# evgueni-ovtchinnikov/raleigh

Hardware: AMD Instinct MI355X
Metric: inner-iter GB/s vs HBM roofline (Gram+dots+SpMM of one block-JCG iteration) (higher is better)
Workload: dtype f64; 1 GPU; block-JCG inner iteration: 9 Gram + 4 dots + 1 SpMM, n=215x215x215=9938375 rows (9938375 per GPU), m=32, 7-pt Laplacian nnz=69291275, rows sharded over 1 GPU(s), strong scaling; n=9938375, m=32, nnz=69291275

## Files before the change

include/rlhip.h:

```cpp
#ifndef RLHIP_H
#define RLHIP_H

#include <stdint.h>

#ifdef __cplusplus
extern "C" {
#endif

#define RLH_VERSION 100

enum { RLH_S = 0, RLH_D = 1, RLH_C = 2, RLH_Z = 3 };

int rlh_version(void);
const char *rlh_last_error(void);
int rlh_device_count(int *count);
int rlh_init(int device);
int rlh_finalize(void);
int rlh_set_stream(void *hip_stream);
int rlh_sync(void);
int rlh_mem_info(int64_t *free_bytes, int64_t *total_bytes);

int rlh_malloc(void **dptr, int64_t bytes);
int rlh_free(void *dptr);
int rlh_memset(void *dptr, int value, int64_t bytes);
int rlh_h2d(void *dptr, const void *hptr, int64_t bytes);
int rlh_d2h(void *hptr, const void *dptr, int64_t bytes);
int rlh_d2d(void *dst, const void *src, int64_t bytes);
int rlh_fetch(void *hptr, const void *dptr, int64_t bytes);
int rlh_copy2d(void *dst, int64_t dpitch, const void *src, int64_t spitch,
               int64_t width_bytes, int64_t rows, int kind);

int rlh_gram(int dtype, int64_t n, int64_t mx, const void *X, int64_t ldx,
             int64_t my, const void *Y, int64_t ldy, void *d_out, void *h_out);

int rlh_gram_multi(int dtype, int64_t n, int nx, const void *const *X, const int64_t *ldx,
                   const int64_t *mx, int ny, const void *const *Y, const int64_t *ldy,
                   const int64_t *my, void *d_out, void *h_out);

int rlh_dots(int dtype, int64_t n, int64_t m, const void *X, int64_t ldx,
             const void *Y, int64_t ldy, void *d_out, void *h_out);

int rlh_dots_transp(int dtype, int64_t n, int64_t m, const void *X, int64_t ldx,
                    const void *Y, int64_t ldy, void *d_out);
int rlh_absmax(int dtype, int64_t n, int64_t m, const void *X, int64_t ldx, double *h_out);

int rlh_block_update(int dtype, int64_t n, int64_t k, const void *X, int64_t ldx,
                     int64_t m, void *Out, int64_t ldo, const void *q,
                     int64_t q_rs, int64_t q_cs, const double *alpha, int beta);

int rlh_block_update2(int dtype, int64_t n, int64_t k1, const void *X1, int64_t ldx1,
                      const void *q1, int64_t q1_rs, int64_t q1_cs, int64_t k2,
                      const void *X2, int64_t ldx2, const void *q2, int64_t q2_rs,
                      int64_t q2_cs, int64_t m, void *Out, int64_t ldo,
                      const double *alpha, int beta);
int rlh_block_update2x2(int dtype, int64_t n, int64_t k1, const void *X1, int64_t ldx1,
                        const void *q1, int64_t q1_rs, int64_t q1_cs, int64_t k2, const void *X2,
                        int64_t ldx2, const void *q2, int64_t q2_rs, int64_t q2_cs, int64_t ma,
                        void *OutA, int64_t ldoa, int64_t mb, void *OutB, int64_t ldob);
int rlh_lincomb_cols(int dtype, int64_t n, int64_t m, const void *a, const void *A,
                     int64_t lda, const void *b, const void *B, int64_t ldb, void *Out,
                     int64_t ldo);
// ... 112 lines not shown
```

raleigh_amd/_lib.py:

```python

import ctypes
import os

import numpy as np

_PKG = os.path.dirname(os.path.abspath(__file__))
LIBPATH = os.path.join(_PKG, 'lib', 'librlhip.so')

RLH_S, RLH_D, RLH_C, RLH_Z = 0, 1, 2, 3

DTYPE_CODE = {np.float32: RLH_S, np.float64: RLH_D, np.complex64: RLH_C, np.complex128: RLH_Z}
DTYPE_SIZE = {np.float32: 4, np.float64: 8, np.complex64: 8, np.complex128: 16}

_i64 = ctypes.c_int64
_p = ctypes.c_void_p
_int = ctypes.c_int

SIGNATURES = {
    'rlh_version': [],
    'rlh_last_error': [],
    'rlh_device_count': [ctypes.POINTER(_int)],
    'rlh_init': [_int],
    'rlh_finalize': [],
    'rlh_set_stream': [_p],
    'rlh_sync': [],
    'rlh_mem_info': [ctypes.POINTER(_i64), ctypes.POINTER(_i64)],
    'rlh_malloc': [ctypes.POINTER(_p), _i64],
    'rlh_free': [_p],
    'rlh_memset': [_p, _int, _i64],
    'rlh_h2d': [_p, _p, _i64],
    'rlh_d2h': [_p, _p, _i64],
    'rlh_d2d': [_p, _p, _i64],
    'rlh_fetch': [_p, _p, _i64],
    'rlh_copy2d': [_p, _i64, _p, _i64, _i64, _i64, _int],
    'rlh_gram': [_int, _i64, _i64, _p, _i64, _i64, _p, _i64, _p, _p],
    'rlh_gram_multi': [_int, _i64, _int, _p, _p, _p, _int, _p, _p, _p, _p, _p],
    'rlh_dots': [_int, _i64, _i64, _p, _i64, _p, _i64, _p, _p],
    'rlh_absmax': [_int, _i64, _i64, _p, _i64, ctypes.POINTER(ctypes.c_double)],
    'rlh_dots_transp': [_int, _i64, _i64, _p, _i64, _p, _i64, _p],
    'rlh_block_update': [_int, _i64, _i64, _p, _i64, _i64, _p, _i64, _p, _i64, _i64, _p, _int],
    'rlh_block_update2': [_int, _i64, _i64, _p, _i64, _p, _i64, _i64, _i64, _p, _i64, _p, _i64, _i64, _i64, _p, _i64,
                          _p, _int],
    'rlh_block_update2x2': [_int, _i64, _i64, _p, _i64, _p, _i64, _i64, _i64, _p, _i64, _p, _i64, _i64, _i64, _p, _i64,
                            _i64, _p, _i64],
    'rlh_lincomb_cols': [_int, _i64, _i64, _p, _p, _i64, _p, _p, _i64, _p, _i64],
    'rlh_axpy': [_int, _i64, _i64, _p, _p, _i64, _p, _i64],
    'rlh_axpy_cols': [_int, _i64, _i64, _p, _p, _i64, _p, _i64],
    'rlh_copy': [_int, _i64, _i64, _p, _i64, _p, _i64],
    'rlh_copy_cols': [_int, _i64, _i64, _p, _p, _i64, _p, _i64],
    'rlh_scale_cols': [_int, _i64, _i64, _p, _int, _p, _i64],
    'rlh_convert': [_int, _int, _i64, _i64, _p, _i64, _p, _i64],
    'rlh_fill_random': [_int, _i64, _i64, _p, _i64, ctypes.c_uint64, _i64, _i64],
    'rlh_conj': [_int, _i64, _i64, _p, _i64],
    'rlh_gather_rows': [_int, _i64, _p, _i64, _p, _i64, _p, _i64],
    'rlh_csr_create': [ctypes.POINTER(_p), _int, _i64, _i64, _p, _p, _p],
    'rlh_csr_create_upper': [ctypes.POINTER(_p), _int, _i64, _p, _p, _p],
    'rlh_csr_destroy': [_p],
    'rlh_csr_info': [_p, ctypes.POINTER(_i64), ctypes.POINTER(_i64), ctypes.POINTER(_i64),
                     ctypes.POINTER(_i64)],
    'rlh_csr_layout': [_p, ctypes.POINTER(_int), ctypes.POINTER(_i64), ctypes.POINTER(ctypes.c_double)],
    'rlh_csr_stacks': [_p, ctypes.POINTER(_i64), ctypes.POINTER(ctypes.c_double), ctypes.POINTER(ctypes.c_double)],
    'rlh_csr_bf16_ready': [_p, _i64, _i64, ctypes.POINTER(_int)],
    'rlh_spmm': [_p, _i64, _p, _i64, _i64, _p, _i64, _p, _i64],
    'rlh_spmm_cheb': [_p, _i64, _p, _i64, _i64, _p, _i64, _p, _i64, _p, _i64, ctypes.c_double, ctypes.c_double,
                      ctypes.c_double],
    'rlh_spmm_part': [_p, _int, _i64, _p, _i64, _i64, _p, _i64, _p, _i64],
# ... 118 lines not shown
```

raleigh_amd/csrc/common.h:

```cpp
#pragma once

#include <hip/hip_runtime.h>
#include <stdint.h>
#include <stdio.h>
#include <string.h>

#include <stdlib.h>

#include <string>
#include <thread>
#include <vector>

#include "rlhip.h"

namespace rlh {

void set_error(const char *fmt, ...);
int hip_fail(hipError_t e, const char *what, const char *file, int line);

#define RLH_HIP(call)                                                   \
  do {                                                                  \
    hipError_t e_ = (call);                                             \
    if (e_ != hipSuccess) return rlh::hip_fail(e_, #call, __FILE__, __LINE__); \
  } while (0)
// ... 64 lines not shown
__device__ __forceinline__ float  add_of(float a, float b)   { return a + b; }
__device__ __forceinline__ double add_of(double a, double b) { return a + b; }
__device__ __forceinline__ c32 add_of(c32 a, c32 b) { return c32{a.re + b.re, a.im + b.im}; }
__device__ __forceinline__ c64 add_of(c64 a, c64 b) { return c64{a.re + b.re, a.im + b.im}; }
__device__ __forceinline__ float  mul_of(float a, float b)   { return a * b; }
__device__ __forceinline__ double mul_of(double a, double b) { return a * b; }
__device__ __forceinline__ c32 mul_of(c32 a, c32 b) { return c32{a.re * b.re - a.im * b.im, a.re * b.im + a.im * b.re}; }
__device__ __forceinline__ c64 mul_of(c64 a, c64 b) { return c64{a.re * b.re - a.im * b.im, a.re * b.im + a.im * b.re}; }

constexpr int kRingSlots = 16;
constexpr size_t kRingSlotBytes = 1u << 20;
constexpr size_t kWorkspaceBytes = 96u << 20;

struct Context {
  bool ready = false;
  int device = -1;
  int num_cu = 256;
  hipStream_t own_stream = nullptr;
  hipStream_t stream = nullptr;
  char *ring_h = nullptr;
  char *ring_d = nullptr;
  hipEvent_t ring_ev[kRingSlots];
  bool ring_used[kRingSlots];
  int ring_next = 0;
  char *work = nullptr;
  char *result_d = nullptr;
  size_t result_d_bytes = 0;
  char *result_h = nullptr;
  char *result_hd = nullptr;
  size_t result_h_bytes = 0;
  hipEvent_t t0 = nullptr, t1 = nullptr;
  unsigned *async_err_h = nullptr;
  unsigned *async_err_d = nullptr;
};

Context &ctx();
int require_ready();
int check_async_error();

int ring_acquire(size_t bytes, int *slot, void **h, void **d);
int ring_commit(int slot, size_t bytes);
int ring_release(int slot);

int ensure_result(size_t bytes);
int fetch_result(void *h_out, const void *d_src, size_t bytes);

static inline bool aligned16(const void *p, int64_t ld, int64_t es) {
  return ((reinterpret_cast<uintptr_t>(p) & 15u) == 0) && (((ld * es) & 15) == 0);
}

}
```

raleigh_amd/csrc/context.hip:

```cpp
#include <stdarg.h>

#include "common.h"

namespace rlh {

static thread_local char g_err[1024] = "";

void set_error(const char *fmt, ...) {
  va_list ap;
  va_start(ap, fmt);
  vsnprintf(g_err, sizeof(g_err), fmt, ap);
  va_end(ap);
}

int hip_fail(hipError_t e, const char *what, const char *file, int line) {
  set_error("hip error %d (%s) in %s at %s:%d", (int)e, hipGetErrorString(e), what, file, line);
  return (int)e ? (int)e : 1;
}

int host_threads() {
  int t = env_int("RLH_HOST_THREADS", 0);
  if (t <= 0) {
    t = (int)std::thread::hardware_concurrency();
    if (t > 16) t = 16;
  }
  return t < 1 ? 1 : t;
}

Context &ctx() {
  static Context c;
  return c;
}

// ... 14 lines not shown
  }
  return 0;
}

int ring_acquire(size_t bytes, int *slot, void **h, void **d) {
  Context &c = ctx();
  RLH_REQUIRE(bytes <= kRingSlotBytes, "coefficient block of %zu bytes exceeds the %zu-byte staging slot",
              bytes, kRingSlotBytes);
  int s = c.ring_next;
  c.ring_next = (s + 1) % kRingSlots;
  if (c.ring_used[s]) RLH_HIP(hipEventSynchronize(c.ring_ev[s]));
  *slot = s;
  *h = c.ring_h + (size_t)s * kRingSlotBytes;
  *d = c.ring_d + (size_t)s * kRingSlotBytes;
  return 0;
}

int ring_commit(int slot, size_t bytes) {
  Context &c = ctx();
  RLH_HIP(hipMemcpyAsync(c.ring_d + (size_t)slot * kRingSlotBytes, c.ring_h + (size_t)slot * kRingSlotBytes,
                         bytes, hipMemcpyHostToDevice, c.stream));
  return 0;
}

int ring_release(int slot) {
  Context &c = ctx();
  RLH_HIP(hipEventRecord(c.ring_ev[slot], c.stream));
  c.ring_used[slot] = true;
  return 0;
}

int ensure_result(size_t bytes) {
  Context &c = ctx();
  if (bytes > c.result_d_bytes) {
    size_t nb = bytes < (1u << 20) ? (1u << 20) : bytes * 2;
    RLH_HIP(hipStreamSynchronize(c.stream));
    if (c.result_d) RLH_HIP(hipFree(c.result_d));
    if (c.result_h) RLH_HIP(hipHostFree(c.result_h));
    c.result_d = nullptr; c.result_h = nullptr; c.result_hd = nullptr; c.result_d_bytes = c.result_h_bytes = 0;
    RLH_HIP(hipMalloc((void **)&c.result_d, nb));
    RLH_HIP(hipHostMalloc((void **)&c.result_h, nb, hipHostMallocMapped));
    RLH_HIP(hipHostGetDevicePointer((void **)&c.result_hd, c.result_h, 0));
    c.result_d_bytes = c.result_h_bytes = nb;
  }
  return 0;
}

int fetch_result(void *h_out, const void *d_src, size_t bytes) {
  Context &c = ctx();
  if (bytes == 0) return 0;
  if (d_src == c.result_hd && bytes <= c.result_h_bytes) {
    RLH_HIP(hipStreamSynchronize(c.stream));
    memcpy(h_out, c.result_h, bytes);
  } else if (bytes <= c.result_h_bytes) {
    RLH_HIP(hipMemcpyAsync(c.result_h, d_src, bytes, hipMemcpyDeviceToHost, c.stream));
    RLH_HIP(hipStreamSynchronize(c.stream));
    memcpy(h_out, c.result_h, bytes);
  } else {
    RLH_HIP(hipMemcpyAsync(h_out, d_src, bytes, hipMemcpyDeviceToHost, c.stream));
    RLH_HIP(hipStreamSynchronize(c.stream));
  }
  return check_async_error();
}

}

using namespace rlh;

extern "C" {

int rlh_version(void) { return RLH_VERSION; }

const char *rlh_last_error(void) { return g_err; }

int rlh_device_count(int *count) {
  RLH_REQUIRE(count != nullptr, "rlh_device_count: null argument");
  RLH_HIP(hipGetDeviceCount(count));
  return 0;
}

int rlh_init(int device) {
  Context &c = ctx();
  if (c.ready) {
    RLH_REQUIRE(c.device == device, "rlh_init: already bound to device %d (one device per process)", c.device);
    return 0;
  }
  int count = 0;
  RLH_HIP(hipGetDeviceCount(&count));
  RLH_REQUIRE(device >= 0 && device < count, "rlh_init: device %d out of range (%d visible)", device, count);
  RLH_HIP(hipSetDevice(device));
  hipDeviceProp_t prop;
  RLH_HIP(hipGetDeviceProperties(&prop, device));
  RLH_REQUIRE(strncmp(prop.gcnArchName, "gfx950", 6) == 0,
              "rlh_init: device %d is %s; this library is built for gfx950 (MI355X) only", device, prop.gcnArchName);
  c.num_cu = prop.multiProcessorCount;
  RLH_HIP(hipStreamCreateWithFlags(&c.own_stream, hipStreamNonBlocking));
  c.stream = c.own_stream;
  RLH_HIP(hipHostMalloc((void **)&c.ring_h, kRingSlots * kRingSlotBytes, hipHostMallocDefault));
  RLH_HIP(hipMalloc((void **)&c.ring_d, kRingSlots * kRingSlotBytes));
  for (int i = 0; i < kRingSlots; ++i) {
    RLH_HIP(hipEventCreateWithFlags(&c.ring_ev[i], hipEventDisableTiming));
    c.ring_used[i] = false;
  }
  RLH_HIP(hipMalloc((void **)&c.work, kWorkspaceBytes));
  RLH_HIP(hipEventCreate(&c.t0));
  RLH_HIP(hipEventCreate(&c.t1));
  RLH_HIP(hipHostMalloc((void **)&c.async_err_h, 64, hipHostMallocMapped));
  *c.async_err_h = 0;
  RLH_HIP(hipHostGetDevicePointer((void **)&c.async_err_d, c.async_err_h, 0));
  c.device = device;
  c.ready = true;
  if (int rc = ensure_result(1u << 20)) return rc;
  return 0;
}

int rlh_finalize(void) {
  Context &c = ctx();
  if (!c.ready) return 0;
  (void)hipStreamSynchronize(c.stream);
  for (int i = 0; i < kRingSlots; ++i) (void)hipEventDestroy(c.ring_ev[i]);
  (void)hipEventDestroy(c.t0);
  (void)hipEventDestroy(c.t1);
  (void)hipHostFree(c.ring_h);
  (void)hipFree(c.ring_d);
  (void)hipFree(c.work);
  if (c.result_d) (void)hipFree(c.result_d);
  if (c.result_h) (void)hipHostFree(c.result_h);
  if (c.async_err_h) (void)hipHostFree(c.async_err_h);
  (void)hipStreamDestroy(c.own_stream);
  c = Context();
  return 0;
}

int rlh_set_stream(void *hip_stream) {
  if (int rc = require_ready()) return rc;
  Context &c = ctx();
  RLH_HIP(hipStreamSynchronize(c.stream));
  c.stream = hip_stream ? (hipStream_t)hip_stream : c.own_stream;
  return 0;
}

int rlh_sync(void) {
  if (int rc = require_ready()) return rc;
  RLH_HIP(hipStreamSynchronize(ctx().stream));
  return check_async_error();
}

int rlh_mem_info(int64_t *free_bytes, int64_t *total_bytes) {
  if (int rc = require_ready()) return rc;
  size_t f = 0, t = 0;
  RLH_HIP(hipMemGetInfo(&f, &t));
  if (free_bytes) *free_bytes = (int64_t)f;
  if (total_bytes) *total_bytes = (int64_t)t;
  return 0;
}

int rlh_malloc(void **dptr, int64_t bytes) {
  if (int rc = require_ready()) return rc;
  RLH_REQUIRE(dptr != nullptr && bytes >= 0, "rlh_malloc: bad arguments");
  *dptr = nullptr;
  if (bytes == 0) return 0;
// ... 8 lines not shown
  RLH_HIP(hipFree(dptr));
  return 0;
}

int rlh_memset(void *dptr, int value, int64_t bytes) {
  if (int rc = require_ready()) return rc;
  if (bytes <= 0) return 0;
  RLH_HIP(hipMemsetAsync(dptr, value, (size_t)bytes, ctx().stream));
  return 0;
}

int rlh_h2d(void *dptr, const void *hptr, int64_t bytes) {
  if (int rc = require_ready()) return rc;
  if (bytes <= 0) return 0;
  RLH_HIP(hipMemcpyAsync(dptr, hptr, (size_t)bytes, hipMemcpyHostToDevice, ctx().stream));
  RLH_HIP(hipStreamSynchronize(ctx().stream));
  return 0;
}

int rlh_d2h(void *hptr, const void *dptr, int64_t bytes) {
  if (int rc = require_ready()) return rc;
  if (bytes <= 0) return 0;
  RLH_HIP(hipMemcpyAsync(hptr, dptr, (size_t)bytes, hipMemcpyDeviceToHost, ctx().stream));
  RLH_HIP(hipStreamSynchronize(ctx().stream));
  return 0;
}

int rlh_fetch(void *hptr, const void *dptr, int64_t bytes) {
  if (int rc = require_ready()) return rc;
  if (bytes <= 0) return 0;
  RLH_REQUIRE(hptr && dptr, "rlh_fetch: null pointer");
  if (int rc = ensure_result((size_t)bytes)) return rc;
  return fetch_result(hptr, dptr, (size_t)bytes);
}

int rlh_d2d(void *dst, const void *src, int64_t bytes) {
  if (int rc = require_ready()) return rc;
  if (bytes <= 0) return 0;
  RLH_HIP(hipMemcpyAsync(dst, src, (size_t)bytes, hipMemcpyDeviceToDevice, ctx().stream));
  return 0;
}

int rlh_copy2d(void *dst, int64_t dpitch, const void *src, int64_t spitch, int64_t width_bytes, int64_t rows,
               int kind) {
  if (int rc = require_ready()) return rc;
  if (width_bytes <= 0 || rows <= 0) return 0;
  RLH_REQUIRE(kind >= 0 && kind <= 2, "rlh_copy2d: kind must be 0 (h2d), 1 (d2h) or 2 (d2d)");
  RLH_REQUIRE(dpitch >= width_bytes && spitch >= width_bytes, "rlh_copy2d: pitch smaller than width");
  hipMemcpyKind k = kind == 0 ? hipMemcpyHostToDevice : (kind == 1 ? hipMemcpyDeviceToHost : hipMemcpyDeviceToDevice);
  RLH_HIP(hipMemcpy2DAsync(dst, (size_t)dpitch, src, (size_t)spitch, (size_t)width_bytes, (size_t)rows, k,
                           ctx().stream));
  if (kind != 2) RLH_HIP(hipStreamSynchronize(ctx().stream));
  return 0;
}

int rlh_timer_start(void) {
  if (int rc = require_ready()) return rc;
  RLH_HIP(hipEventRecord(ctx().t0, ctx().stream));
  return 0;
}

int rlh_timer_stop(float *milliseconds) {
  if (int rc = require_ready()) return rc;
  RLH_HIP(hipEventRecord(ctx().t1, ctx().stream));
  RLH_HIP(hipEventSynchronize(ctx().t1));
  float ms = 0.f;
// ... 7 lines not shown
```

raleigh_amd/csrc/gram.hip:

```cpp
#include <stdlib.h>

#include "common.h"

namespace rlh {

template <typename R> struct Mfma16;
template <> struct Mfma16<double> {
  typedef double acc_t __attribute__((ext_vector_type(4)));
  static __device__ __forceinline__ acc_t run(double a, double b, acc_t c) {
    return __builtin_amdgcn_mfma_f64_16x16x4f64(a, b, c, 0, 0, 0);
  }
  static __device__ __forceinline__ int out_row(int lane, int reg) { return (lane >> 4) + 4 * reg; }
};
template <> struct Mfma16<float> {
  typedef float acc_t __attribute__((ext_vector_type(4)));
  static __device__ __forceinline__ acc_t run(float a, float b, acc_t c) {
    return __builtin_amdgcn_mfma_f32_16x16x4f32(a, b, c, 0, 0, 0);
  }
  static __device__ __forceinline__ int out_row(int lane, int reg) { return (lane >> 4) * 4 + reg; }
};

struct GramSeg { const void *p; int64_t ld; int c0; };
constexpr int kGramSegs = 4;

// ... 400 lines not shown
      const double fa0 = *reinterpret_cast<const double *>(base + ya0 + ro + k8);
      const double fa1 = *reinterpret_cast<const double *>(base + ya1 + ro + k8);
      const double fb = *reinterpret_cast<const double *>(base + xo + ro + k8);
      const double fj = sgn * *reinterpret_cast<const double *>(base + xo + ro + k8j);
      acc[0][0] = __builtin_amdgcn_mfma_f64_16x16x4f64(fa0, fb, acc[0][0], 0, 0, 0);
      acc[1][0] = __builtin_amdgcn_mfma_f64_16x16x4f64(fa1, fb, acc[1][0], 0, 0, 0);
      acc[0][1] = __builtin_amdgcn_mfma_f64_16x16x4f64(fa0, fj, acc[0][1], 0, 0, 0);
      acc[1][1] = __builtin_amdgcn_mfma_f64_16x16x4f64(fa1, fj, acc[1][1], 0, 0, 0);
    }
  }
  __syncthreads();
  acc_t *red = reinterpret_cast<acc_t *>(zlds);
  if (grp == 1) {
#pragma unroll
    for (int t = 0; t < 4; ++t) red[(u * 4 + t) * 64 + lane] = acc[t >> 1][t & 1];
  }
  __syncthreads();
  if (grp == 0) {
#pragma unroll
    for (int t = 0; t < 4; ++t) {
      const acc_t o = red[(u * 4 + t) * 64 + lane];
      const acc_t v = acc[t >> 1][t & 1];
      const int ti = 2 * yp + (t >> 1);
      const int jj = (t & 1) * 64 + xj * 16 + (lane & 15);
#pragma unroll
      for (int r = 0; r < 4; ++r) {
        const int ii = ti * 16 + (lane >> 4) + 4 * r;
        a.partials[(int64_t)(ii * 128 + jj) * gridDim.x + blockIdx.x] = v[r] + o[r];
      }
    }
  }
}

__global__ __launch_bounds__(256) void gram_z_finalize(const double *partials, int nb, int my, int mx, c64 *out) {
  const int lane = threadIdx.x & 63;
  const int e = blockIdx.x * 4 + (threadIdx.x >> 6);
  if (e >= my * mx) return;
  const int i = e / mx, j = e % mx;
  const double *pr = partials + (int64_t)(i * 128 + j) * nb, *pi = partials + (int64_t)(i * 128 + 64 + j) * nb;
  double sr = 0.0, si = 0.0;
  for (int b = lane; b < nb; b += 64) { sr += pr[b]; si += pi[b]; }
#pragma unroll
  for (int off = 32; off > 0; off >>= 1) { sr += __shfl_xor(sr, off); si += __shfl_xor(si, off); }
  if (lane == 0) out[e] = c64{sr, si};
}

static int gram_z_dma_launch(int64_t n, int64_t mx, const void *X, int64_t ldx, int64_t my, const void *Y, int64_t ldy,
                             void *d_out) {
  Context &c = ctx();
  ZGramArgs a;
  a.X = (const c64 *)X; a.Y = (const c64 *)Y; a.ldx = ldx; a.ldy = ldy; a.n = n; a.mx = (int)mx; a.my = (int)my;
  a.nchunks = (n + kZgRows - 1) / kZgRows;
  a.partials = (double *)c.work;
  int64_t nb = c.num_cu;
  if (nb > a.nchunks) nb = a.nchunks;
  RLH_REQUIRE((size_t)nb * 64 * 128 * sizeof(double) <= kWorkspaceBytes, "rlh_gram: reduction workspace");
#define RLH_ZG(D_)                                                                                                  \
  do {                                                                                                              \
    static bool attr = false;                                                                                       \
    if (!attr) {                                                                                                    \
      RLH_HIP(hipFuncSetAttribute(reinterpret_cast<const void *>(&gram_z_dma_kernel<D_>),                           \
                                  hipFuncAttributeMaxDynamicSharedMemorySize, 2 * kZgBuf));                         \
      attr = true;                                                                                                  \
    }                                                                                                               \
    hipLaunchKernelGGL(gram_z_dma_kernel<D_>, dim3((unsigned)nb), dim3(1024), 2 * kZgBuf, c.stream, a);             \
  } while (0)
  switch (getenv("RLH_GRAM_ZDBG") ? atoi(getenv("RLH_GRAM_ZDBG")) : 0) {
    case 1: RLH_ZG(1); break;
    case 2: RLH_ZG(2); break;
    case 3: RLH_ZG(3); break;
    default: RLH_ZG(0); break;
  }
#undef RLH_ZG
  RLH_HIP(hipGetLastError());
  const int total = (int)(my * mx);
  hipLaunchKernelGGL(gram_z_finalize, dim3((total + 3) / 4), dim3(256), 0, c.stream, (const double *)c.work, (int)nb, (int)my,
                     (int)mx, (c64 *)d_out);
  RLH_HIP(hipGetLastError());
  return 0;
}

template <int DT>
__global__ __launch_bounds__(256) void gram_finalize(const void *partials_, int nbx, int npj, int VY, int VX, int my,
                                                     int mx, void *out_, int same) {
  using T = typename DType<DT>::T;
  using R = typename DType<DT>::R;
  constexpr bool CPLX = DType<DT>::cplx;
  constexpr int NCOMP = CPLX ? 4 : 1;
  const R *partials = reinterpret_cast<const R *>(partials_);
  const int lane = threadIdx.x & 63;
  const int e = blockIdx.x * 4 + (threadIdx.x >> 6);
  if (e >= my * mx) return;
  const int i = e / mx, j = e % mx;
  const int64_t slab = (int64_t)VY * VX;
  double t[NCOMP];
#pragma unroll
  for (int comp = 0; comp < NCOMP; ++comp) {
    int vi = CPLX ? 2 * i + (comp >> 1) : i;
    int vj = CPLX ? 2 * j + (comp & 1) : j;
    if (same && vi / VY == vj / VX && (vi % VY) / 16 > (vj % VX) / 16) { const int t_ = vi; vi = vj; vj = t_; }
    const int panel = (vi / VY) * npj + (vj / VX);
    const R *p = partials + ((int64_t)panel * slab + (vi % VY) * VX + (vj % VX)) * nbx;
    double s = 0.0;
    for (int b = lane; b < nbx; b += 64) s += (double)p[b];
#pragma unroll
    for (int off = 32; off > 0; off >>= 1) s += __shfl_xor(s, off);
    t[comp] = s;
  }
  if (lane == 0) {
    T *out = reinterpret_cast<T *>(out_);
    if constexpr (!CPLX) {
      out[e] = (R)t[0];
    } else {
      out[e].re = (R)(t[0] + t[3]);
      out[e].im = (R)(t[1] - t[2]);
    }
  }
}

template <int DT, int PI, int PJ, bool ALIGNED, int MODE, bool MULTI = false, bool QUAD = false, bool SYMS = false>
static int gram_blocks_per_cu() {
  static int cached = 0;
  if (cached == 0) {
    int nb = 0;
    if (hipOccupancyMaxActiveBlocksPerMultiprocessor(&nb, gram_kernel<DT, PI, PJ, ALIGNED, MODE, MULTI, QUAD, SYMS>, QUAD ? 512 : 256, 0) != hipSuccess ||
        nb < 1)
      nb = 1;
    cached = nb > 8 ? 8 : nb;
    const char *e = getenv("RLH_GRAM_WG_PER_CU");
    if (e && *e && atoi(e) > 0 && atoi(e) < cached) cached = atoi(e);
  }
  return cached;
}

static inline bool env_quad() {
  const char *e = getenv("RLH_GRAM_QUAD");
  return !(e && *e == '0');
}

static inline int pick_tiles(int v) {
  if (v <= 16) return 1;
  if (v <= 32) return 2;
  return 4;
}

template <int DT, int PI, int PJ, bool ALIGNED, int MODE, bool MULTI = false, bool QUAD = false, bool SYMS = false>
static int gram_launch(GramArgs &a, int npi, int npj, int64_t my, int64_t mx, void *d_out) {
  using R = typename DType<DT>::R;
  Context &c = ctx();
  constexpr int VY = PI * 16 * (QUAD ? 2 : 1), VX = PJ * 16 * (QUAD ? 4 : 1);
  const int npanels = npi * npj;
  int64_t nbx = (int64_t)c.num_cu * gram_blocks_per_cu<DT, PI, PJ, ALIGNED, MODE, MULTI, QUAD, SYMS>() / npanels;
  if (nbx < 1) nbx = 1;
  if (nbx > a.nchunks) nbx = a.nchunks;
  const size_t part_bytes = sizeof(R) * VY * VX;
  while (nbx > 1 && (size_t)nbx * npanels * part_bytes > kWorkspaceBytes) nbx /= 2;
  RLH_REQUIRE((size_t)nbx * npanels * part_bytes <= kWorkspaceBytes,
              "rlh_gram: %lld x %lld result exceeds the reduction workspace", (long long)my, (long long)mx);
  hipLaunchKernelGGL((gram_kernel<DT, PI, PJ, ALIGNED, MODE, MULTI, QUAD, SYMS>), dim3((unsigned)nbx, (unsigned)npanels), dim3(QUAD ? 512 : 256), 0,
                     c.stream, a);
  RLH_HIP(hipGetLastError());
  const int total = (int)(my * mx);
  hipLaunchKernelGGL((gram_finalize<DT>), dim3((total + 3) / 4), dim3(256), 0, c.stream, c.work, (int)nbx, npj, VY,
                     VX, (int)my, (int)mx, d_out, a.same);
  RLH_HIP(hipGetLastError());
  return 0;
}

static int gram_nt(int64_t bytes) {
  const char *e = getenv("RLH_GRAM_NT");
  if (e && *e) return atoi(e);
  return bytes > (int64_t)192 << 20;
}

constexpr int gram_stream_waves(int ncol) { return ncol <= 16 ? 16 : (ncol <= 32 ? 8 : 4); }

template <typename R, int TB, int NYC, int NXC, bool NT, bool XAL = false, bool CPLX = false>
__global__ __launch_bounds__(64 * (XAL ? 8 : gram_stream_waves(NYC + NXC))) void gram_stream_kernel(GramArgs a) {
  using M = Mfma16<R>;
  using acc_t = typename M::acc_t;
  constexpr bool SELF = NYC == 0;
  constexpr int RPU = 16 / (int)sizeof(R);
  constexpr int NP = TB / 16;
  constexpr int ROWS = NP * RPU;
  constexpr int NCOL = XAL ? NYC : NYC + NXC;
  constexpr int NC = CPLX ? 2 : 1;
  constexpr int NPT = NP * NC;
  constexpr int CPL = 64 / NPT;
  constexpr int NL = NCOL / NC / CPL;
  static_assert(!(CPLX && XAL) && NPT <= 64, "complex tiles");
  constexpr int KS = ROWS / 4;
  constexpr int SW = NP / 16;
  constexpr int PJ = NXC / 16, PI = SELF ? PJ : NYC / 16;
  static_assert(NP >= 16 && NP <= 64 && 64 % NP == 0 && NCOL % CPL == 0, "tile shape");
  constexpr int WPG = XAL ? 8 : gram_stream_waves(NYC + NXC);
  extern __shared__ __attribute__((aligned(16))) char lds_all[];
  char *lds = lds_all + (threadIdx.x >> 6) * (NCOL * TB);
// ... 212 lines not shown
    lds = (size_t)8 * 64 * TB;
    if (lds < (size_t)8 * 8 * 256 * sizeof(R)) lds = (size_t)8 * 8 * 256 * sizeof(R);
    if (lds < 84 * 1024) lds = 84 * 1024;
    nbx = c.num_cu;
    if (nbx * 8 > ntiles) nbx = (ntiles + 7) / 8;
    if (nbx < 1) nbx = 1;
    nparts_alias = nbx;
#define RLH_GSA(NT_)                                                                                                   \
  do {                                                                                                                 \
    static bool attr = false;                                                                                          \
    if (!attr) {                                                                                                       \
      RLH_HIP(hipFuncSetAttribute(reinterpret_cast<const void *>(&gram_stream_kernel<R, TB, 64, 32, NT_, true>),       \
                                  hipFuncAttributeMaxDynamicSharedMemorySize, 160 * 1024));                            \
      attr = true;                                                                                                     \
    }                                                                                                                  \
    hipLaunchKernelGGL((gram_stream_kernel<R, TB, 64, 32, NT_, true>), dim3((unsigned)nbx), dim3(64 * 8),                    \
                       lds, c.stream, a);                                                                              \
  } while (0)
    if (a.nt & 1) RLH_GSA(true); else RLH_GSA(false);
#undef RLH_GSA
  } else if (nxc == 16) {
    if (nyc == 0) RLH_GS(0, 16); else if (nyc == 16) RLH_GS(16, 16); else if (nyc == 32) RLH_GS(32, 16); else RLH_GS(64, 16);
  } else if (nxc == 32) {
    if (nyc == 0) RLH_GS(0, 32); else if (nyc == 16) RLH_GS(16, 32); else if (nyc == 32) RLH_GS(32, 32); else RLH_GS(64, 32);
  } else {
    if (nyc == 0) RLH_GS(0, 64); else RLH_GS(64, 64);
  }
#undef RLH_GS
#undef RLH_GS1
  RLH_HIP(hipGetLastError());
  const int total = (int)(my * mx);
  hipLaunchKernelGGL((gram_finalize<DT>), dim3((total + 3) / 4), dim3(256), 0, c.stream, c.work,
                     (int)(nparts_alias ? nparts_alias : nparts), 1, VY, nxc,
                     (int)my, (int)mx, d_out, a.same);
  RLH_HIP(hipGetLastError());
  return 0;
}

template <int DT>
static int gram_impl(int64_t n, int64_t mx, const void *X, int64_t ldx, int64_t my, const void *Y, int64_t ldy,
                     void *d_out) {
  using R = typename DType<DT>::R;
  constexpr int NC = DType<DT>::cplx ? 2 : 1;
  Context &c = ctx();
  const int vx = (int)mx * NC, vy = (int)my * NC;
  const int PI = pick_tiles(vy), PJ = pick_tiles(vx);
  const int npi = (vy + PI * 16 - 1) / (PI * 16), npj = (vx + PJ * 16 - 1) / (PJ * 16);
  GramArgs a;
  a.X = X; a.Y = Y; a.ldx = ldx; a.ldy = ldy; a.n = n; a.mx = (int)mx; a.my = (int)my;
  a.same = (X == Y && ldx == ldy && mx == my) ? 1 : 0;
  a.npj = npj; a.partials = c.work;
  const int64_t es = dtype_size(DT);
  a.nt = gram_nt(n * (a.same ? mx : mx + my) * es);
  const bool aligned = aligned16(X, ldx, es) && aligned16(Y, ldy, es);
  {
    const int stream = getenv("RLH_GRAM_STREAM") ? atoi(getenv("RLH_GRAM_STREAM")) : 1;
    if (stream && aligned && vx <= 64 && vy <= 64 && (vx > 8 || vy > 8)) {
      a.npj = 1;
      a.xal = -1;
      a.nxs = a.nys = 1;
      a.xs[0] = GramSeg{X, ldx, 0};
      a.ys[0] = GramSeg{Y, ldy, 0};
      for (int k = 1; k < kGramSegs; ++k) a.xs[k] = a.ys[k] = GramSeg{nullptr, 0, 1 << 30};
      return gram_stream_launch<DT>(a, my, mx, d_out);
    }
  }
  static const int pipe = getenv("RLH_GRAM_PIPE") ? atoi(getenv("RLH_GRAM_PIPE")) : 1;
// ... 133 lines not shown
      for (int i = 0; i < 4; ++i)
#pragma unroll
        for (int e = 0; e < VEC; ++e) fma_conj_acc(acc, xv[i].v[e], xv[i].v[e]);
    } else if (ALIGNED && base + 4 * 256 * VEC <= n) {
      V xv[4], yv[4];
#pragma unroll
      for (int i = 0; i < 4; ++i) {
        const int64_t r = base + ((int64_t)i * 256 + threadIdx.x) * VEC;
        xv[i] = piece(x + r);
        yv[i] = piece(y + r);
      }
#pragma unroll
      for (int i = 0; i < 4; ++i)
#pragma unroll
        for (int e = 0; e < VEC; ++e) fma_conj_acc(acc, yv[i].v[e], xv[i].v[e]);
    } else {
      for (int i = 0; i < 4; ++i) {
        const int64_t r = base + ((int64_t)i * 256 + threadIdx.x) * VEC;
        for (int e = 0; e < VEC && r + e < n; ++e) fma_conj_acc(acc, y[r + e], x[r + e]);
      }
    }
  }
  __shared__ T red[256];
  red[threadIdx.x] = acc;
  __syncthreads();
  for (int s = 128; s > 0; s >>= 1) {
    if (threadIdx.x < s) red[threadIdx.x] = add_of(red[threadIdx.x], red[threadIdx.x + s]);
    __syncthreads();
  }
  if (threadIdx.x == 0) partials[(int64_t)col * nbx + blockIdx.x] = red[0];
}

template <typename T>
__global__ __launch_bounds__(256) void dots_finalize(const T *partials, int nbx, int m, T *out) {
  const int lane = threadIdx.x & 63;
  const int col = blockIdx.x * 4 + (threadIdx.x >> 6);
  if (col >= m) return;
  T s = zero_of(T{});
  for (int b = lane; b < nbx; b += 64) s = add_of(s, partials[(int64_t)col * nbx + b]);
  if constexpr (sizeof(T) == sizeof(float) || sizeof(T) == sizeof(double)) {
    using R = T;
#pragma unroll
    for (int off = 32; off > 0; off >>= 1) s = s + (R)__shfl_xor(s, off);
  }
  if (lane == 0) out[col] = s;
}

template <typename R2, typename C>
__device__ __forceinline__ C shfl_complex(C v, int off) {
  C r;
  r.re = __shfl_xor(v.re, off);
  r.im = __shfl_xor(v.im, off);
  return r;
}

template <>
__global__ __launch_bounds__(256) void dots_finalize<c32>(const c32 *partials, int nbx, int m, c32 *out) {
  const int lane = threadIdx.x & 63;
  const int col = blockIdx.x * 4 + (threadIdx.x >> 6);
  if (col >= m) return;
  c32 s = zero_of(c32{});
  for (int b = lane; b < nbx; b += 64) s = add_of(s, partials[(int64_t)col * nbx + b]);
#pragma unroll
  for (int off = 32; off > 0; off >>= 1) s = add_of(s, shfl_complex<float>(s, off));
  if (lane == 0) out[col] = s;
}

template <>
__global__ __launch_bounds__(256) void dots_finalize<c64>(const c64 *partials, int nbx, int m, c64 *out) {
  const int lane = threadIdx.x & 63;
  const int col = blockIdx.x * 4 + (threadIdx.x >> 6);
  if (col >= m) return;
  c64 s = zero_of(c64{});
  for (int b = lane; b < nbx; b += 64) s = add_of(s, partials[(int64_t)col * nbx + b]);
#pragma unroll
  for (int off = 32; off > 0; off >>= 1) s = add_of(s, shfl_complex<double>(s, off));
  if (lane == 0) out[col] = s;
}

template <int DT>
static int dots_impl(int64_t n, int64_t m, const void *X, int64_t ldx, const void *Y, int64_t ldy, void *d_out) {
  using T = typename DType<DT>::T;
  Context &c = ctx();
  constexpr int VEC = 16 / (int)sizeof(T);
  int per = 4;
  int64_t nbx = (n + 256 * VEC * (int64_t)per - 1) / (256 * VEC * (int64_t)per);
  while (nbx > 2048 || (nbx > 1 && (size_t)nbx * m * sizeof(T) > kWorkspaceBytes / 4)) {
    per += 4;
    nbx = (n + 256 * VEC * (int64_t)per - 1) / (256 * VEC * (int64_t)per);
  }
  if (nbx < 1) nbx = 1;
  RLH_REQUIRE((size_t)nbx * m * sizeof(T) <= kWorkspaceBytes, "rlh_dots: too many columns");
  const int nt = gram_nt(n * m * (int64_t)sizeof(T) * (X == Y ? 1 : 2));
  const bool aligned = aligned16(X, ldx, sizeof(T)) && aligned16(Y, ldy, sizeof(T));
  dim3 grid((unsigned)nbx, (unsigned)m);
  if (aligned && (nt & 1))
    hipLaunchKernelGGL((dots_kernel<T, true, true>), grid, dim3(256), 0, c.stream, (const T *)X, ldx, (const T *)Y, ldy,
                       n, (T *)c.work, (int)nbx, per);
  else if (aligned)
    hipLaunchKernelGGL((dots_kernel<T, true, false>), grid, dim3(256), 0, c.stream, (const T *)X, ldx, (const T *)Y, ldy,
                       n, (T *)c.work, (int)nbx, per);
  else
    hipLaunchKernelGGL((dots_kernel<T, false, false>), grid, dim3(256), 0, c.stream, (const T *)X, ldx, (const T *)Y, ldy,
                       n, (T *)c.work, (int)nbx, per);
  RLH_HIP(hipGetLastError());
  hipLaunchKernelGGL((dots_finalize<T>), dim3(((int)m + 3) / 4), dim3(256), 0, c.stream, (const T *)c.work,
                     (int)nbx, (int)m, (T *)d_out);
  RLH_HIP(hipGetLastError());
  return 0;
}

template <typename R>
__global__ __launch_bounds__(256) void absmax_kernel(const R *X, int64_t ldx_r, int64_t n_r, double *partials, int nbx) {
  const R *x = X + (int64_t)blockIdx.y * ldx_r;
  double mx = 0.0;
  const int64_t stride = (int64_t)gridDim.x * 256;
  for (int64_t r = (int64_t)blockIdx.x * 256 + threadIdx.x; r < n_r; r += stride) {
    const double v = fabs((double)x[r]);
    mx = v > mx ? v : mx;
  }
  __shared__ double red[256];
  red[threadIdx.x] = mx;
  __syncthreads();
  for (int s = 128; s > 0; s >>= 1) {
    if (threadIdx.x < s) red[threadIdx.x] = red[threadIdx.x] > red[threadIdx.x + s] ? red[threadIdx.x] : red[threadIdx.x + s];
    __syncthreads();
  }
  if (threadIdx.x == 0) partials[(int64_t)blockIdx.y * nbx + blockIdx.x] = red[0];
}

__global__ __launch_bounds__(256) void absmax_finalize(const double *partials, int64_t count, double *out) {
  double mx = 0.0;
  for (int64_t i = threadIdx.x; i < count; i += 256) mx = partials[i] > mx ? partials[i] : mx;
  __shared__ double red[256];
  red[threadIdx.x] = mx;
  __syncthreads();
  for (int s = 128; s > 0; s >>= 1) {
    if (threadIdx.x < s) red[threadIdx.x] = red[threadIdx.x] > red[threadIdx.x + s] ? red[threadIdx.x] : red[threadIdx.x + s];
    __syncthreads();
  }
  if (threadIdx.x == 0) out[0] = red[0];
}

template <int DT>
static int absmax_impl(int64_t n, int64_t m, const void *X, int64_t ldx, void *d_out) {
  using R = typename DType<DT>::R;
  constexpr int NC = DType<DT>::cplx ? 2 : 1;
  Context &c = ctx();
  int64_t nbx = (n * NC + 256 * 8 - 1) / (256 * 8);
  const int64_t cap = ((int64_t)c.num_cu * 8 + m - 1) / m;
  if (nbx > cap) nbx = cap;
  if (nbx < 1) nbx = 1;
  RLH_REQUIRE((size_t)nbx * m * sizeof(double) <= kWorkspaceBytes, "rlh_absmax: too many columns");
  hipLaunchKernelGGL((absmax_kernel<R>), dim3((unsigned)nbx, (unsigned)m), dim3(256), 0, c.stream, (const R *)X,
                     ldx * NC, n * NC, (double *)c.work, (int)nbx);
  RLH_HIP(hipGetLastError());
  hipLaunchKernelGGL(absmax_finalize, dim3(1), dim3(256), 0, c.stream, (const double *)c.work, nbx * m, (double *)d_out);
  RLH_HIP(hipGetLastError());
  return 0;
}

template <typename T>
__global__ __launch_bounds__(256) void dots_transp_kernel(const T *X, int64_t ldx, const T *Y, int64_t ldy,
                                                          int64_t n, int m, T *out) {
  const int64_t stride = (int64_t)gridDim.x * blockDim.x;
  for (int64_t r = (int64_t)blockIdx.x * blockDim.x + threadIdx.x; r < n; r += stride) {
    T acc = zero_of(T{});
    for (int i = 0; i < m; ++i) fma_conj_acc(acc, Y[r + (int64_t)i * ldy], X[r + (int64_t)i * ldx]);
    out[r] = acc;
  }
}

template <int DT>
static int dots_transp_impl(int64_t n, int64_t m, const void *X, int64_t ldx, const void *Y, int64_t ldy,
                            void *d_out) {
  using T = typename DType<DT>::T;
  Context &c = ctx();
  int64_t nb = (n + 255) / 256;
  if (nb > (int64_t)c.num_cu * 8) nb = (int64_t)c.num_cu * 8;
  hipLaunchKernelGGL((dots_transp_kernel<T>), dim3((unsigned)nb), dim3(256), 0, c.stream, (const T *)X, ldx,
                     (const T *)Y, ldy, n, (int)m, (T *)d_out);
  RLH_HIP(hipGetLastError());
  return 0;
}

}

using namespace rlh;

#define RLH_DISPATCH(dt, fn, ...)                              \
// ... 126 lines not shown
```

Baseline: 6338 GB/s.

## Publish reduction completion via mapped host word and poll instead of stream sync

Finalize kernels for gram, dots and absmax now do a grid-wide atomic counter, and the last block writes a sequence number into a mapped host word. When the result lands in the mapped host buffer, fetch_result spin-polls that word, falling back to hipStreamSynchronize on timeout. The goal is to avoid stream-sync latency on small reductions that return to the host. The dots finalize also unrolls its strided partial sum. The cost is CPU spinning, extra atomics in every finalize, and subtle memory-ordering risk.

```diff
diff --git a/include/rlhip.h b/include/rlhip.h
--- a/include/rlhip.h
+++ b/include/rlhip.h
@@ -27,6 +27,7 @@
 int rlh_d2h(void *hptr, const void *dptr, int64_t bytes);
 int rlh_d2d(void *dst, const void *src, int64_t bytes);
 int rlh_fetch(void *hptr, const void *dptr, int64_t bytes);
+int rlh_poll_word(const void *word, uint32_t expect, int64_t timeout_us);
 int rlh_copy2d(void *dst, int64_t dpitch, const void *src, int64_t spitch,
                int64_t width_bytes, int64_t rows, int kind);
 
diff --git a/raleigh_amd/_lib.py b/raleigh_amd/_lib.py
--- a/raleigh_amd/_lib.py
+++ b/raleigh_amd/_lib.py
@@ -32,6 +32,7 @@
     'rlh_d2h': [_p, _p, _i64],
     'rlh_d2d': [_p, _p, _i64],
     'rlh_fetch': [_p, _p, _i64],
+    'rlh_poll_word': [_p, ctypes.c_uint32, _i64],
     'rlh_copy2d': [_p, _i64, _p, _i64, _i64, _i64, _int],
     'rlh_gram': [_int, _i64, _i64, _p, _i64, _i64, _p, _i64, _p, _p],
     'rlh_gram_multi': [_int, _i64, _int, _p, _p, _p, _int, _p, _p, _p, _p, _p],
diff --git a/raleigh_amd/csrc/common.h b/raleigh_amd/csrc/common.h
--- a/raleigh_amd/csrc/common.h
+++ b/raleigh_amd/csrc/common.h
@@ -120,7 +120,34 @@
   hipEvent_t t0 = nullptr, t1 = nullptr;
   unsigned *async_err_h = nullptr;
   unsigned *async_err_d = nullptr;
+  unsigned *pub_word_h = nullptr;
+  unsigned *pub_word_d = nullptr;
+  unsigned *pub_count_d = nullptr;
+  unsigned pub_seq = 0;
+  unsigned pub_expect = 0;
 };
+
+struct Publish {
+  unsigned *seq = nullptr;
+  unsigned *count = nullptr;
+  unsigned value = 0;
+};
+
+#if defined(__HIP__)
+__device__ __forceinline__ void publish_done(const Publish &p) {
+  if (p.seq == nullptr) return;
+  __builtin_amdgcn_fence(__ATOMIC_RELEASE, "");
+  __syncthreads();
+  if (threadIdx.x == 0) {
+    const unsigned total = gridDim.x * gridDim.y * gridDim.z;
+    const unsigned prev = __hip_atomic_fetch_add(p.count, 1u, __ATOMIC_ACQ_REL, __HIP_MEMORY_SCOPE_AGENT);
+    if (prev == total - 1) {
+      __hip_atomic_store(p.count, 0u, __ATOMIC_RELAXED, __HIP_MEMORY_SCOPE_AGENT);
+      __hip_atomic_store(p.seq, p.value, __ATOMIC_RELEASE, __HIP_MEMORY_SCOPE_SYSTEM);
+    }
+  }
+}
+#endif
 
 Context &ctx();
 int require_ready();
@@ -131,7 +158,9 @@
 int ring_release(int slot);
 
 int ensure_result(size_t bytes);
+Publish publish_for(const void *d_out);
 int fetch_result(void *h_out, const void *d_src, size_t bytes);
+bool poll_word(const volatile unsigned *word, unsigned expect, int64_t timeout_us);
 
 static inline bool aligned16(const void *p, int64_t ld, int64_t es) {
   return ((reinterpret_cast<uintptr_t>(p) & 15u) == 0) && (((ld * es) & 15) == 0);
diff --git a/raleigh_amd/csrc/context.hip b/raleigh_amd/csrc/context.hip
--- a/raleigh_amd/csrc/context.hip
+++ b/raleigh_amd/csrc/context.hip
@@ -1,4 +1,7 @@
 #include <stdarg.h>
+
+#include <atomic>
+#include <chrono>
 
 #include "common.h"
 
@@ -79,25 +82,62 @@
 
 int ensure_result(size_t bytes) {
   Context &c = ctx();
+  c.pub_expect = 0;
   if (bytes > c.result_d_bytes) {
     size_t nb = bytes < (1u << 20) ? (1u << 20) : bytes * 2;
     RLH_HIP(hipStreamSynchronize(c.stream));
     if (c.result_d) RLH_HIP(hipFree(c.result_d));
     if (c.result_h) RLH_HIP(hipHostFree(c.result_h));
     c.result_d = nullptr; c.result_h = nullptr; c.result_hd = nullptr; c.result_d_bytes = c.result_h_bytes = 0;
+    c.pub_word_h = c.pub_word_d = nullptr;
     RLH_HIP(hipMalloc((void **)&c.result_d, nb));
-    RLH_HIP(hipHostMalloc((void **)&c.result_h, nb, hipHostMallocMapped));
+    RLH_HIP(hipHostMalloc((void **)&c.result_h, nb + 64, hipHostMallocMapped));
     RLH_HIP(hipHostGetDevicePointer((void **)&c.result_hd, c.result_h, 0));
     c.result_d_bytes = c.result_h_bytes = nb;
-  }
-  return 0;
+    c.pub_word_h = reinterpret_cast<unsigned *>(c.result_h + nb);
+    c.pub_word_d = reinterpret_cast<unsigned *>(c.result_hd + nb);
+    *(volatile unsigned *)c.pub_word_h = 0;
+  }
+  return 0;
+}
+
+Publish publish_for(const void *d_out) {
+  Context &c = ctx();
+  Publish p;
+  const char *o = static_cast<const char *>(d_out);
+  if (!c.pub_word_d || !c.pub_count_d || o < c.result_hd || o >= c.result_hd + c.result_h_bytes) return p;
+  if (++c.pub_seq == 0) ++c.pub_seq;
+  p.seq = c.pub_word_d;
+  p.count = c.pub_count_d;
+  p.value = c.pub_seq;
+  c.pub_expect = c.pub_seq;
+  return p;
+}
+
+bool poll_word(const volatile unsigned *word, unsigned expect, int64_t timeout_us) {
+  const auto t0 = std::chrono::steady_clock::now();
+  for (unsigned i = 0;; ++i) {
+    if (*word == expect) {
+      std::atomic_thread_fence(std::memory_order_acquire);
+      return true;
+    }
+    if ((i & 63) == 63 &&
+        std::chrono::steady_clock::now() - t0 > std::chrono::microseconds(timeout_us < 0 ? 0 : timeout_us))
+      return false;
+#if defined(__x86_64__) || defined(__i386__)
+    __builtin_ia32_pause();
+#endif
+  }
 }
 
 int fetch_result(void *h_out, const void *d_src, size_t bytes) {
   Context &c = ctx();
   if (bytes == 0) return 0;
   if (d_src == c.result_hd && bytes <= c.result_h_bytes) {
-    RLH_HIP(hipStreamSynchronize(c.stream));
+    const unsigned expect = c.pub_expect;
+    c.pub_expect = 0;
+    const int64_t budget = env_int("RLH_FETCH_POLL_US", 20000);
+    if (!(expect != 0 && budget > 0 && poll_word(c.pub_word_h, expect, budget))) RLH_HIP(hipStreamSynchronize(c.stream));
     memcpy(h_out, c.result_h, bytes);
   } else if (bytes <= c.result_h_bytes) {
     RLH_HIP(hipMemcpyAsync(c.result_h, d_src, bytes, hipMemcpyDeviceToHost, c.stream));
@@ -155,6 +195,8 @@
   RLH_HIP(hipHostMalloc((void **)&c.async_err_h, 64, hipHostMallocMapped));
   *c.async_err_h = 0;
   RLH_HIP(hipHostGetDevicePointer((void **)&c.async_err_d, c.async_err_h, 0));
+  RLH_HIP(hipMalloc((void **)&c.pub_count_d, 64));
+  RLH_HIP(hipMemset(c.pub_count_d, 0, 64));
   c.device = device;
   c.ready = true;
   if (int rc = ensure_result(1u << 20)) return rc;
@@ -174,6 +216,7 @@
   if (c.result_d) (void)hipFree(c.result_d);
   if (c.result_h) (void)hipHostFree(c.result_h);
   if (c.async_err_h) (void)hipHostFree(c.async_err_h);
+  if (c.pub_count_d) (void)hipFree(c.pub_count_d);
   (void)hipStreamDestroy(c.own_stream);
   c = Context();
   return 0;
@@ -248,6 +291,11 @@
   RLH_REQUIRE(hptr && dptr, "rlh_fetch: null pointer");
   if (int rc = ensure_result((size_t)bytes)) return rc;
   return fetch_result(hptr, dptr, (size_t)bytes);
+}
+
+int rlh_poll_word(const void *word, uint32_t expect, int64_t timeout_us) {
+  if (!word) return 0;
+  return poll_word(static_cast<const volatile unsigned *>(word), expect, timeout_us) ? 1 : 0;
 }
 
 int rlh_d2d(void *dst, const void *src, int64_t bytes) {
diff --git a/raleigh_amd/csrc/gram.hip b/raleigh_amd/csrc/gram.hip
--- a/raleigh_amd/csrc/gram.hip
+++ b/raleigh_amd/csrc/gram.hip
@@ -456,17 +456,20 @@
   }
 }
 
-__global__ __launch_bounds__(256) void gram_z_finalize(const double *partials, int nb, int my, int mx, c64 *out) {
+__global__ __launch_bounds__(256) void gram_z_finalize(const double *partials, int nb, int my, int mx, c64 *out,
+                                                       Publish pub) {
   const int lane = threadIdx.x & 63;
   const int e = blockIdx.x * 4 + (threadIdx.x >> 6);
-  if (e >= my * mx) return;
-  const int i = e / mx, j = e % mx;
-  const double *pr = partials + (int64_t)(i * 128 + j) * nb, *pi = partials + (int64_t)(i * 128 + 64 + j) * nb;
-  double sr = 0.0, si = 0.0;
-  for (int b = lane; b < nb; b += 64) { sr += pr[b]; si += pi[b]; }
-#pragma unroll
-  for (int off = 32; off > 0; off >>= 1) { sr += __shfl_xor(sr, off); si += __shfl_xor(si, off); }
-  if (lane == 0) out[e] = c64{sr, si};
+  if (e < my * mx) {
+    const int i = e / mx, j = e % mx;
+    const double *pr = partials + (int64_t)(i * 128 + j) * nb, *pi = partials + (int64_t)(i * 128 + 64 + j) * nb;
+    double sr = 0.0, si = 0.0;
+    for (int b = lane; b < nb; b += 64) { sr += pr[b]; si += pi[b]; }
+#pragma unroll
+    for (int off = 32; off > 0; off >>= 1) { sr += __shfl_xor(sr, off); si += __shfl_xor(si, off); }
+    if (lane == 0) out[e] = c64{sr, si};
+  }
+  publish_done(pub);
 }
 
 static int gram_z_dma_launch(int64_t n, int64_t mx, const void *X, int64_t ldx, int64_t my, const void *Y, int64_t ldy,
@@ -499,14 +502,14 @@
   RLH_HIP(hipGetLastError());
   const int total = (int)(my * mx);
   hipLaunchKernelGGL(gram_z_finalize, dim3((total + 3) / 4), dim3(256), 0, c.stream, (const double *)c.work, (int)nb, (int)my,
-                     (int)mx, (c64 *)d_out);
+                     (int)mx, (c64 *)d_out, publish_for(d_out));
   RLH_HIP(hipGetLastError());
   return 0;
 }
 
 template <int DT>
-__global__ __launch_bounds__(256) void gram_finalize(const void *partials_, int nbx, int npj, int VY, int VX, int my,
-                                                     int mx, void *out_, int same) {
+__device__ __forceinline__ void gram_finalize_entry(const void *partials_, int nbx, int npj, int VY, int VX, int my,
+                                                    int mx, void *out_, int same) {
   using T = typename DType<DT>::T;
   using R = typename DType<DT>::R;
   constexpr bool CPLX = DType<DT>::cplx;
@@ -540,6 +543,13 @@
       out[e].im = (R)(t[1] - t[2]);
     }
   }
+}
+
+template <int DT>
+__global__ __launch_bounds__(256) void gram_finalize(const void *partials_, int nbx, int npj, int VY, int VX, int my,
+                                                     int mx, void *out_, int same, Publish pub) {
+  gram_finalize_entry<DT>(partials_, nbx, npj, VY, VX, my, mx, out_, same);
+  publish_done(pub);
 }
 
 template <int DT, int PI, int PJ, bool ALIGNED, int MODE, bool MULTI = false, bool QUAD = false, bool SYMS = false>
@@ -586,7 +596,7 @@
   RLH_HIP(hipGetLastError());
   const int total = (int)(my * mx);
   hipLaunchKernelGGL((gram_finalize<DT>), dim3((total + 3) / 4), dim3(256), 0, c.stream, c.work, (int)nbx, npj, VY,
-                     VX, (int)my, (int)mx, d_out, a.same);
+                     VX, (int)my, (int)mx, d_out, a.same, publish_for(d_out));
   RLH_HIP(hipGetLastError());
   return 0;
 }
@@ -865,7 +875,7 @@
   const int total = (int)(my * mx);
   hipLaunchKernelGGL((gram_finalize<DT>), dim3((total + 3) / 4), dim3(256), 0, c.stream, c.work,
                      (int)(nparts_alias ? nparts_alias : nparts), 1, VY, nxc,
-                     (int)my, (int)mx, d_out, a.same);
+                     (int)my, (int)mx, d_out, a.same, publish_for(d_out));
   RLH_HIP(hipGetLastError());
   return 0;
 }
@@ -1065,18 +1075,34 @@
 }
 
 template <typename T>
-__global__ __launch_bounds__(256) void dots_finalize(const T *partials, int nbx, int m, T *out) {
+__device__ __forceinline__ T strided_lane_sum(const T *p, int lane, int nbx) {
+  constexpr int U = 16;
+  T s = zero_of(T{});
+  for (int b0 = lane; b0 < nbx; b0 += 64 * U) {
+    T t[U];
+#pragma unroll
+    for (int k = 0; k < U; ++k) t[k] = b0 + 64 * k < nbx ? p[b0 + 64 * k] : zero_of(T{});
+#pragma unroll
+    for (int k = 0; k < U; ++k)
+      if (b0 + 64 * k < nbx) s = add_of(s, t[k]);
+  }
+  return s;
+}
+
+template <typename T>
+__global__ __launch_bounds__(256) void dots_finalize(const T *partials, int nbx, int m, T *out, Publish pub) {
   const int lane = threadIdx.x & 63;
   const int col = blockIdx.x * 4 + (threadIdx.x >> 6);
-  if (col >= m) return;
-  T s = zero_of(T{});
-  for (int b = lane; b < nbx; b += 64) s = add_of(s, partials[(int64_t)col * nbx + b]);
-  if constexpr (sizeof(T) == sizeof(float) || sizeof(T) == sizeof(double)) {
-    using R = T;
-#pragma unroll
-    for (int off = 32; off > 0; off >>= 1) s = s + (R)__shfl_xor(s, off);
-  }
-  if (lane == 0) out[col] = s;
+  if (col < m) {
+    T s = strided_lane_sum(partials + (int64_t)col * nbx, lane, nbx);
+    if constexpr (sizeof(T) == sizeof(float) || sizeof(T) == sizeof(double)) {
+      using R = T;
+#pragma unroll
+      for (int off = 32; off > 0; off >>= 1) s = s + (R)__shfl_xor(s, off);
+    }
+    if (lane == 0) out[col] = s;
+  }
+  publish_done(pub);
 }
 
 template <typename R2, typename C>
@@ -1088,27 +1114,29 @@
 }
 
 template <>
-__global__ __launch_bounds__(256) void dots_finalize<c32>(const c32 *partials, int nbx, int m, c32 *out) {
+__global__ __launch_bounds__(256) void dots_finalize<c32>(const c32 *partials, int nbx, int m, c32 *out, Publish pub) {
   const int lane = threadIdx.x & 63;
   const int col = blockIdx.x * 4 + (threadIdx.x >> 6);
-  if (col >= m) return;
-  c32 s = zero_of(c32{});
-  for (int b = lane; b < nbx; b += 64) s = add_of(s, partials[(int64_t)col * nbx + b]);
-#pragma unroll
-  for (int off = 32; off > 0; off >>= 1) s = add_of(s, shfl_complex<float>(s, off));
-  if (lane == 0) out[col] = s;
+  if (col < m) {
+    c32 s = strided_lane_sum(partials + (int64_t)col * nbx, lane, nbx);
+#pragma unroll
+    for (int off = 32; off > 0; off >>= 1) s = add_of(s, shfl_complex<float>(s, off));
+    if (lane == 0) out[col] = s;
+  }
+  publish_done(pub);
 }
 
 template <>
-__global__ __launch_bounds__(256) void dots_finalize<c64>(const c64 *partials, int nbx, int m, c64 *out) {
+__global__ __launch_bounds__(256) void dots_finalize<c64>(const c64 *partials, int nbx, int m, c64 *out, Publish pub) {
   const int lane = threadIdx.x & 63;
   const int col = blockIdx.x * 4 + (threadIdx.x >> 6);
-  if (col >= m) return;
-  c64 s = zero_of(c64{});
-  for (int b = lane; b < nbx; b += 64) s = add_of(s, partials[(int64_t)col * nbx + b]);
-#pragma unroll
-  for (int off = 32; off > 0; off >>= 1) s = add_of(s, shfl_complex<double>(s, off));
-  if (lane == 0) out[col] = s;
+  if (col < m) {
+    c64 s = strided_lane_sum(partials + (int64_t)col * nbx, lane, nbx);
+#pragma unroll
+    for (int off = 32; off > 0; off >>= 1) s = add_of(s, shfl_complex<double>(s, off));
+    if (lane == 0) out[col] = s;
+  }
+  publish_done(pub);
 }
 
 template <int DT>
@@ -1138,7 +1166,7 @@
                        n, (T *)c.work, (int)nbx, per);
   RLH_HIP(hipGetLastError());
   hipLaunchKernelGGL((dots_finalize<T>), dim3(((int)m + 3) / 4), dim3(256), 0, c.stream, (const T *)c.work,
-                     (int)nbx, (int)m, (T *)d_out);
+                     (int)nbx, (int)m, (T *)d_out, publish_for(d_out));
   RLH_HIP(hipGetLastError());
   return 0;
 }
@@ -1162,7 +1190,7 @@
   if (threadIdx.x == 0) partials[(int64_t)blockIdx.y * nbx + blockIdx.x] = red[0];
 }
 
-__global__ __launch_bounds__(256) void absmax_finalize(const double *partials, int64_t count, double *out) {
+__global__ __launch_bounds__(256) void absmax_finalize(const double *partials, int64_t count, double *out, Publish pub) {
   double mx = 0.0;
   for (int64_t i = threadIdx.x; i < count; i += 256) mx = partials[i] > mx ? partials[i] : mx;
   __shared__ double red[256];
@@ -1173,6 +1201,7 @@
     __syncthreads();
   }
   if (threadIdx.x == 0) out[0] = red[0];
+  publish_done(pub);
 }
 
 template <int DT>
@@ -1188,7 +1217,8 @@
   hipLaunchKernelGGL((absmax_kernel<R>), dim3((unsigned)nbx, (unsigned)m), dim3(256), 0, c.stream, (const R *)X,
                      ldx * NC, n * NC, (double *)c.work, (int)nbx);
   RLH_HIP(hipGetLastError());
-  hipLaunchKernelGGL(absmax_finalize, dim3(1), dim3(256), 0, c.stream, (const double *)c.work, nbx * m, (double *)d_out);
+  hipLaunchKernelGGL(absmax_finalize, dim3(1), dim3(256), 0, c.stream, (const double *)c.work, nbx * m, (double *)d_out,
+                     publish_for(d_out));
   RLH_HIP(hipGetLastError());
   return 0;
 }
```

Measured after the change: 6320 GB/s (median of 2 runs). Within noise of the previous version (-0.3%).
